# ChocoWu/SeTok

Measured on AMD Instinct MI355X. Metric: images/s SeTok encode (ViT-L/14, 224^2, dyn-k), higher is better.
Workload: dtype bf16; 1 GPU; cfg2: ViT-L/14 224^2 (24 of 24 layers, select_layer=-1 as the reference's launch scripts pass it), dyn-k DPC-kNN (k=64, threshold=0.125), SeTok head 1024/2 heads/ff 4096 -> 4096, mm_in_projector mlp2x_gelu; encode-only; batch_per_gpu=256, global_batch=256, slowest_rank=0

## Files before the change

setok_amd/csrc/attn_seg.hip:

```cpp
#include "lds_mma.h"

namespace {

constexpr int SD = 512;
constexpr int WD = 128;
constexpr int VROW = WD * 2;

__device__ __forceinline__ void attn_seg_big_segment(const bf16* __restrict__ qkv, const int32_t* __restrict__ seg_offsets, bf16* __restrict__ out, int H,
                                                     float scale_log2e, const int s, const int h, float (*Sp)[16 * 64], char (*Vs)[32 * VROW]) {
    const int tid = threadIdx.x, lane = tid & 63;
    const int wave = __builtin_amdgcn_readfirstlane(tid >> 6);
    const int r0 = seg_offsets[s];
    const int n = seg_offsets[s + 1] - r0;
    if (n <= 32) return;
    const int nt = (n + 31) >> 5;
    const int64_t C = (int64_t)H * SD, ld = 3 * C;
    const bf16* qb = qkv + (int64_t)r0 * ld + h * SD + wave * WD;
    const bf16* kb = qb + C;
    const bf16* vb = qb + 2 * C;
    const int qi = lane & 31, hi = lane >> 5;
    const int g16 = lane >> 4, i16 = lane & 15;
    const int tr_row = (i16 >> 2) + 4 * (g16 >> 1);
    const int tr_col = (g16 & 1) * 16 + (i16 & 3) * 4;
    const unsigned vlds = __builtin_amdgcn_readfirstlane((unsigned)(size_t)(__attribute__((address_space(3))) char*)&Vs[0][0]) + wave * (32 * VROW);
    float* mySp = &Sp[wave][0];

    for (int qt = 0; qt < nt; ++qt) {
        const int q = qt * 32 + qi;
        const bf16* qp = qb + (int64_t)min(q, n - 1) * ld + hi * 8;
        bf16x8 qf[8];
#pragma unroll
        for (int ks = 0; ks < 8; ++ks) qf[ks] = *reinterpret_cast<const bf16x8*>(qp + ks * 16);
        f32x16 o[4];
#pragma unroll
        for (int d = 0; d < 4; ++d)
#pragma unroll
            for (int r = 0; r < 16; ++r) o[d][r] = 0.f;
        float m_run = -INFINITY, l_run = 0.f;

        for (int kt = 0; kt < nt; ++kt) {
#pragma unroll
            for (int i = 0; i < 8; ++i) {
                const int p = i * 64 + lane, key = kt * 32 + (p >> 4), c = p & 15;
                const bf16* src = vb + (int64_t)min(key, n - 1) * ld + c * 8;
                lds_dma16(src, vlds + i * 1024);
            }
            f32x16 sp;
#pragma unroll
            for (int r = 0; r < 16; ++r) sp[r] = 0.f;
            const bf16* kp = kb + (int64_t)min(kt * 32 + qi, n - 1) * ld + hi * 8;
            bf16x8 kf[8];
#pragma unroll
            for (int ks = 0; ks < 8; ++ks) kf[ks] = *reinterpret_cast<const bf16x8*>(kp + ks * 16);
#pragma unroll
            for (int ks = 0; ks < 8; ++ks) sp = __builtin_amdgcn_mfma_f32_32x32x16_bf16(kf[ks], qf[ks], sp, 0, 0, 0);
#pragma unroll
            for (int r = 0; r < 16; ++r) mySp[r * 64 + lane] = sp[r];
            __syncthreads();
            float t[16];
#pragma unroll
            for (int r = 0; r < 16; ++r) t[r] = (Sp[0][r * 64 + lane] + Sp[1][r * 64 + lane]) + (Sp[2][r * 64 + lane] + Sp[3][r * 64 + lane]);
            __syncthreads();
            float mx = -INFINITY;
            const bool tail = (kt == nt - 1) && (n & 31);
#pragma unroll
            for (int r = 0; r < 16; ++r) {
                if (tail) { const int key = kt * 32 + (r & 3) + 8 * (r >> 2) + 4 * hi; if (key >= n) t[r] = -INFINITY; }
                mx = fmaxf(mx, t[r]);
            }
            mx = fmaxf(mx, __shfl_xor(mx, 32, 64));
            const float m_new = fmaxf(m_run, mx);
            if (!__all(m_new == m_run)) {
                const float alpha = __builtin_amdgcn_exp2f((m_run - m_new) * scale_log2e);
                l_run *= alpha;
#pragma unroll
                for (int d = 0; d < 4; ++d)
#pragma unroll
                    for (int r = 0; r < 16; ++r) o[d][r] *= alpha;
                m_run = m_new;
            }
            const float mc = m_run * scale_log2e;
            float ls = 0.f;
#pragma unroll
            for (int r = 0; r < 16; ++r) { t[r] = __builtin_amdgcn_exp2f(fmaf(t[r], scale_log2e, -mc)); ls += t[r]; }
            l_run += ls;
            const bf16x8 p0 = pack8(t), p1 = pack8(t + 8);
            asm volatile("s_waitcnt vmcnt(0)" ::: "memory");
            const char* Vw = &Vs[wave][0];
#pragma unroll
            for (int d = 0; d < 4; ++d) {
#pragma unroll
                for (int k2 = 0; k2 < 2; ++k2) {
                    const char* va = Vw + (k2 * 16 + tr_row) * VROW + (d * 32 + tr_col) * 2;
                    o[d] = __builtin_amdgcn_mfma_f32_32x32x16_bf16(lds_read_tr16(va, va + 8 * VROW), k2 == 0 ? p0 : p1, o[d], 0, 0, 0);
                }
            }
            asm volatile("s_waitcnt lgkmcnt(0)" ::: "memory");
        }
        const float l_tot = l_run + __shfl_xor(l_run, 32, 64);
        const float inv = 1.0f / l_tot;
        if (q < n) {
            bf16* op = out + ((int64_t)r0 + q) * C + h * SD + wave * WD;
#pragma unroll
            for (int d = 0; d < 4; ++d)
#pragma unroll
                for (int r4 = 0; r4 < 4; ++r4) {
                    bf16x4 v;
#pragma unroll
                    for (int j = 0; j < 4; ++j) v[j] = (bf16)(o[d][r4 * 4 + j] * inv);
                    *reinterpret_cast<bf16x4*>(op + d * 32 + 8 * r4 + 4 * hi) = v;
                }
        }
    }
}

template <int SPW>
__global__ __launch_bounds__(256) void attn_seg_big_kernel(const bf16* __restrict__ qkv, const int32_t* __restrict__ seg_offsets, int n_segs,
                                                           bf16* __restrict__ out, int H, float scale_log2e) {
    __shared__ __attribute__((aligned(16))) float Sp[4][16 * 64];
    __shared__ __attribute__((aligned(16))) char Vs[4][32 * VROW];
    if constexpr (SPW == 1) {
        attn_seg_big_segment(qkv, seg_offsets, out, H, scale_log2e, blockIdx.x, blockIdx.y, Sp, Vs);
    } else {
        static_assert(SPW == 64, "one lane per segment length");
        const int sl = blockIdx.x * 64 + (threadIdx.x & 63);
        const int nl = sl < n_segs ? seg_offsets[sl + 1] - seg_offsets[sl] : 0;
        unsigned long long m = __ballot(nl > 32);
        while (m) {
            const int b = __builtin_amdgcn_readfirstlane(__ffsll((long long)m) - 1);
            m &= m - 1;
            attn_seg_big_segment(qkv, seg_offsets, out, H, scale_log2e, blockIdx.x * 64 + b, blockIdx.y, Sp, Vs);
            __syncthreads();
        }
    }
}

__global__ __launch_bounds__(256) void attn_seg_small_kernel(const bf16* __restrict__ qkv, const int32_t* __restrict__ seg_offsets, int n_segs,
                                                             bf16* __restrict__ out, int H, float scale_log2e) {
    __shared__ __attribute__((aligned(16))) char Vs[4][32 * VROW];
    const int tid = threadIdx.x, lane = tid & 63;
    const int wave = __builtin_amdgcn_readfirstlane(tid >> 6);
    const int s = blockIdx.x * 4 + wave, h = blockIdx.y;
    if (s >= n_segs) return;
    const int r0 = seg_offsets[s];
    const int n = seg_offsets[s + 1] - r0;
    if (n <= 0 || n > 32) return;
    const int64_t C = (int64_t)H * SD, ld = 3 * C;
    const bf16* qb = qkv + (int64_t)r0 * ld + h * SD;
    const int qi = lane & 31, hi = lane >> 5;
    const int g16 = lane >> 4, i16 = lane & 15;
    const int tr_row = (i16 >> 2) + 4 * (g16 >> 1);
    const int tr_col = (g16 & 1) * 16 + (i16 & 3) * 4;
    const unsigned vlds = __builtin_amdgcn_readfirstlane((unsigned)(size_t)(__attribute__((address_space(3))) char*)&Vs[0][0]) + wave * (32 * VROW);
    const bf16* rowp = qb + (int64_t)min(qi, n - 1) * ld + hi * 8;
    float t[16];
#pragma unroll
    for (int r = 0; r < 16; ++r) t[r] = 0.f;
    f32x16 part[4];
#pragma unroll
    for (int w = 0; w < 4; ++w) {
        bf16x8 qf[8], kf[8];
#pragma unroll
        for (int ks = 0; ks < 8; ++ks) {
            qf[ks] = *reinterpret_cast<const bf16x8*>(rowp + w * WD + ks * 16);
            kf[ks] = *reinterpret_cast<const bf16x8*>(rowp + C + w * WD + ks * 16);
        }
#pragma unroll
        for (int r = 0; r < 16; ++r) part[w][r] = 0.f;
#pragma unroll
        for (int ks = 0; ks < 8; ++ks) part[w] = __builtin_amdgcn_mfma_f32_32x32x16_bf16(kf[ks], qf[ks], part[w], 0, 0, 0);
    }
    float mx = -INFINITY;
#pragma unroll
    for (int r = 0; r < 16; ++r) {
        t[r] = (part[0][r] + part[1][r]) + (part[2][r] + part[3][r]);
        const int key = (r & 3) + 8 * (r >> 2) + 4 * hi;
        if (key >= n) t[r] = -INFINITY;
        mx = fmaxf(mx, t[r]);
    }
    mx = fmaxf(mx, __shfl_xor(mx, 32, 64));
    const float mc = mx * scale_log2e;
    float ls = 0.f;
#pragma unroll
    for (int r = 0; r < 16; ++r) { t[r] = __builtin_amdgcn_exp2f(fmaf(t[r], scale_log2e, -mc)); ls += t[r]; }
    const float inv = 1.0f / (ls + __shfl_xor(ls, 32, 64));
    const bf16x8 p0 = pack8(t), p1 = pack8(t + 8);
    const char* Vw = &Vs[wave][0];
#pragma unroll 1
    for (int w = 0; w < 4; ++w) {
        const bf16* vb = qb + 2 * C + w * WD;
#pragma unroll
        for (int i = 0; i < 8; ++i) {
            const int p = i * 64 + lane, key = p >> 4, c = p & 15;
            const bf16* src = vb + (int64_t)min(key, n - 1) * ld + c * 8;
            lds_dma16(src, vlds + i * 1024);
        }
        asm volatile("s_waitcnt vmcnt(0)" ::: "memory");
        f32x16 o[4];
#pragma unroll
        for (int d = 0; d < 4; ++d) {
#pragma unroll
            for (int r = 0; r < 16; ++r) o[d][r] = 0.f;
#pragma unroll
            for (int k2 = 0; k2 < 2; ++k2) {
                const char* va = Vw + (k2 * 16 + tr_row) * VROW + (d * 32 + tr_col) * 2;
                o[d] = __builtin_amdgcn_mfma_f32_32x32x16_bf16(lds_read_tr16(va, va + 8 * VROW), k2 == 0 ? p0 : p1, o[d], 0, 0, 0);
            }
        }
        asm volatile("s_waitcnt lgkmcnt(0)" ::: "memory");
        if (qi < n) {
            bf16* op = out + ((int64_t)r0 + qi) * C + h * SD + w * WD;
#pragma unroll
            for (int d = 0; d < 4; ++d)
#pragma unroll
                for (int r4 = 0; r4 < 4; ++r4) {
                    bf16x4 v;
#pragma unroll
                    for (int j = 0; j < 4; ++j) v[j] = (bf16)(o[d][r4 * 4 + j] * inv);
                    *reinterpret_cast<bf16x4*>(op + d * 32 + 8 * r4 + 4 * hi) = v;
                }
        }
    }
}

}

int setok_attention_seg_bf16(hipStream_t s, const bf16* qkv, const int32_t* seg_offsets, int n_segs, int max_len, bf16* out, int rows, int H, int Dh, float scale) {
    if (Dh != SD || !seg_offsets || n_segs <= 0 || rows <= 0) return SETOK_EUNSUPPORTED;
    attn_seg_small_kernel<<<dim3(cdiv(n_segs, 4), H), 256, 0, s>>>(qkv, seg_offsets, n_segs, out, H, scale * 1.44269504088896340736f);
    if (max_len > 32) {
        if (n_segs > 2048) attn_seg_big_kernel<64><<<dim3(cdiv(n_segs, 64), H), 256, 0, s>>>(qkv, seg_offsets, n_segs, out, H, scale * 1.44269504088896340736f);
        else attn_seg_big_kernel<1><<<dim3(n_segs, H), 256, 0, s>>>(qkv, seg_offsets, n_segs, out, H, scale * 1.44269504088896340736f);
    }
    SETOK_CHECK_LAUNCH("setok_attention(segments bf16)");
    return SETOK_OK;
}
```

Before: 6345 images/s.

## Restructure small-segment attention with LDS-staged Q/K/V, swizzled layout, persistent grid

Rewrites the small-segment (n<=32) attention kernel to be persistent, with each wave looping over segments picked by ballot from a strided set. Segments of 8 or 16 tokens are handled by a staged path that DMAs Q, K and V rows into XOR-swizzled LDS. Outputs are staged through LDS so global writes are coalesced 16-byte stores, and V loads are overlapped with compute. The goal is to cut wasted loads for short segments, bank conflicts and uncoalesced stores, at the cost of much more complex code, 24KB of LDS per wave, and occupancy pinned at 2 waves per EU.

```diff
diff --git a/setok_amd/csrc/attn_seg.hip b/setok_amd/csrc/attn_seg.hip
--- a/setok_amd/csrc/attn_seg.hip
+++ b/setok_amd/csrc/attn_seg.hip
@@ -135,27 +135,186 @@
     }
 }
 
-__global__ __launch_bounds__(256) void attn_seg_small_kernel(const bf16* __restrict__ qkv, const int32_t* __restrict__ seg_offsets, int n_segs,
-                                                             bf16* __restrict__ out, int H, float scale_log2e) {
-    __shared__ __attribute__((aligned(16))) char Vs[4][32 * VROW];
-    const int tid = threadIdx.x, lane = tid & 63;
-    const int wave = __builtin_amdgcn_readfirstlane(tid >> 6);
-    const int s = blockIdx.x * 4 + wave, h = blockIdx.y;
-    if (s >= n_segs) return;
-    const int r0 = seg_offsets[s];
-    const int n = seg_offsets[s + 1] - r0;
-    if (n <= 0 || n > 32) return;
-    const int64_t C = (int64_t)H * SD, ld = 3 * C;
-    const bf16* qb = qkv + (int64_t)r0 * ld + h * SD;
-    const int qi = lane & 31, hi = lane >> 5;
+constexpr int SMALL_LDS = 24 * 1024;
+
+__device__ __forceinline__ int seg_swz(int row) { return ((row & 3) << 2) | ((row >> 2) & 3); }
+
+template <int NR>
+__device__ __forceinline__ void seg_stage(const char* base, int64_t ldb, int n, unsigned dst, int lane) {
+    constexpr int RPR = NR / 8, LPR = 64 / RPR;
+    const int rl = lane / LPR, pc = lane % LPR;
+#pragma unroll
+    for (int j = 0; j < 8; ++j) {
+        if (j * RPR < n) {
+            const int row = j * RPR + rl;
+            lds_dma16(base + (int64_t)min(row, n - 1) * ldb + ((pc ^ seg_swz(row)) << 4), dst + j * 1024);
+        }
+    }
+}
+
+template <int P, int KS>
+__device__ __forceinline__ void seg_pv(const char* Vb, int sb, int n, int lane, bf16x8 p0, bf16x8 p1, f32x16 (&o)[4]) {
     const int g16 = lane >> 4, i16 = lane & 15;
     const int tr_row = (i16 >> 2) + 4 * (g16 >> 1);
-    const int tr_col = (g16 & 1) * 16 + (i16 & 3) * 4;
-    const unsigned vlds = __builtin_amdgcn_readfirstlane((unsigned)(size_t)(__attribute__((address_space(3))) char*)&Vs[0][0]) + wave * (32 * VROW);
+    const int colb = (g16 & 1) * 32 + (i16 & 3) * 8;
+    const char* ra[KS][2];
+    int sw[KS][2];
+#pragma unroll
+    for (int k2 = 0; k2 < KS; ++k2)
+#pragma unroll
+        for (int u = 0; u < 2; ++u) {
+            const int r = min(k2 * 16 + tr_row + 8 * u, n - 1);
+            ra[k2][u] = Vb + r * P;
+            sw[k2][u] = seg_swz(r);
+        }
+#pragma unroll
+    for (int d = 0; d < 4; ++d) {
+#pragma unroll
+        for (int r = 0; r < 16; ++r) o[d][r] = 0.f;
+        const int b = sb + d * 64 + colb;
+#pragma unroll
+        for (int k2 = 0; k2 < KS; ++k2) {
+            const char* a0 = ra[k2][0] + ((((b >> 4) ^ sw[k2][0]) << 4) | (b & 8));
+            const char* a1 = ra[k2][1] + ((((b >> 4) ^ sw[k2][1]) << 4) | (b & 8));
+            o[d] = __builtin_amdgcn_mfma_f32_32x32x16_bf16(lds_read_tr16(a0, a1), k2 == 0 ? p0 : p1, o[d], 0, 0, 0);
+        }
+    }
+}
+
+template <int PO>
+__device__ __forceinline__ void seg_o_write(const f32x16 (&o)[4], float inv, char* Ob, int sb, int qi, int hi, bool live) {
+    if (live) {
+        char* orow = Ob + qi * PO;
+        const int z = seg_swz(qi);
+#pragma unroll
+        for (int d = 0; d < 4; ++d)
+#pragma unroll
+            for (int r4 = 0; r4 < 4; ++r4) {
+                bf16x4 v;
+#pragma unroll
+                for (int j = 0; j < 4; ++j) v[j] = (bf16)(o[d][r4 * 4 + j] * inv);
+                const int cb = sb + d * 64 + r4 * 16;
+                *reinterpret_cast<bf16x4*>(orow + ((((cb >> 4) ^ z) << 4) | (hi * 8))) = v;
+            }
+    }
+}
+
+template <int PO, int NR>
+__device__ __forceinline__ void seg_o_flush(const char* Ob, bf16* op, int64_t C, int n, int lane) {
+    constexpr int LPR = PO / 16, RPS = 64 / LPR;
+    const int rl = lane / LPR, pc = lane % LPR;
+#pragma unroll
+    for (int j = 0; j < NR / RPS; ++j) {
+        if (j * RPS < n) {
+            const int row = j * RPS + rl;
+            if (row < n) {
+                const bf16x8 v = *reinterpret_cast<const bf16x8*>(Ob + row * PO + ((pc ^ seg_swz(row)) << 4));
+                *reinterpret_cast<bf16x8*>(op + (int64_t)row * C + pc * 8) = v;
+            }
+        }
+    }
+}
+
+template <int LIVE>
+__device__ __forceinline__ float seg_softmax(float* t, int n, int hi, float scale_log2e) {
+    float mx = -INFINITY;
+#pragma unroll
+    for (int r = 0; r < LIVE; ++r) {
+        const int key = (r & 3) + 8 * (r >> 2) + 4 * hi;
+        if (key >= n) t[r] = -INFINITY;
+        mx = fmaxf(mx, t[r]);
+    }
+    mx = fmaxf(mx, __shfl_xor(mx, 32, 64));
+    const float mc = mx * scale_log2e;
+    float ls = 0.f;
+#pragma unroll
+    for (int r = 0; r < LIVE; ++r) { t[r] = __builtin_amdgcn_exp2f(fmaf(t[r], scale_log2e, -mc)); ls += t[r]; }
+#pragma unroll
+    for (int r = LIVE; r < 16; ++r) t[r] = 0.f;
+    return 1.0f / (ls + __shfl_xor(ls, 32, 64));
+}
+
+template <int NR>
+__device__ __forceinline__ void attn_seg_small_staged(const bf16* qb, bf16* ob, int n, int64_t C, float scale_log2e, unsigned lds, char* Lw, int lane) {
+    const char* L = Lw;
+    constexpr int R = NR / 8, SPR = 4 / R, P = SPR * VROW;
+    constexpr unsigned QO = 0, KO = 8192, VO = 16384;
+    const int64_t ldb = 6 * C;
+    const char* qbytes = reinterpret_cast<const char*>(qb);
+    const int qi = lane & 31, hi = lane >> 5;
+    seg_stage<NR>(qbytes, ldb, n, lds + QO, lane);
+    seg_stage<NR>(qbytes + 2 * C, ldb, n, lds + KO, lane);
+    seg_stage<NR>(qbytes + 4 * C, ldb, n, lds + VO, lane);
+    const int row = min(qi, n - 1);
+    const char* fq = L + QO + row * P;
+    const int fz = seg_swz(row);
+    f32x16 part[4];
+#pragma unroll
+    for (int g = 0; g < R; ++g) {
+        asm volatile("s_waitcnt vmcnt(0)" ::: "memory");
+#pragma unroll
+        for (int wl = 0; wl < SPR; ++wl) {
+            const int w = g * SPR + wl;
+            bf16x8 qf[8], kf[8];
+#pragma unroll
+            for (int ks = 0; ks < 8; ++ks) {
+                const int c = ((wl * 16 + ks * 2 + hi) ^ fz) << 4;
+                qf[ks] = *reinterpret_cast<const bf16x8*>(fq + c);
+                kf[ks] = *reinterpret_cast<const bf16x8*>(fq + (KO - QO) + c);
+            }
+#pragma unroll
+            for (int r = 0; r < 16; ++r) part[w][r] = 0.f;
+#pragma unroll
+            for (int ks = 0; ks < 8; ++ks) part[w] = __builtin_amdgcn_mfma_f32_32x32x16_bf16(kf[ks], qf[ks], part[w], 0, 0, 0);
+        }
+        if (R > 1) {
+            asm volatile("s_waitcnt lgkmcnt(0)" ::: "memory");
+            if (g + 1 < R) {
+                seg_stage<NR>(qbytes + (g + 1) * P, ldb, n, lds + QO, lane);
+                seg_stage<NR>(qbytes + 2 * C + (g + 1) * P, ldb, n, lds + KO, lane);
+            } else {
+                seg_stage<NR>(qbytes + 4 * C + P, ldb, n, lds + QO, lane);
+            }
+        }
+    }
+    float t[16];
+#pragma unroll
+    for (int r = 0; r < NR / 2; ++r) t[r] = (part[0][r] + part[1][r]) + (part[2][r] + part[3][r]);
+    const float inv = seg_softmax<NR / 2>(t, n, hi, scale_log2e);
+    const bf16x8 p0 = pack8(t), p1 = pack8(t + 8);
+    const bool live = qi < n;
+    if constexpr (R == 1) {
+#pragma unroll
+        for (int w = 0; w < 4; ++w) {
+            f32x16 o[4];
+            seg_pv<P, 1>(L + VO, w * VROW, n, lane, p0, p1, o);
+            seg_o_write<1024>(o, inv, Lw + QO, w * VROW, qi, hi, live);
+        }
+        seg_o_flush<1024, 8>(L + QO, ob, C, n, lane);
+    } else {
+        f32x16 o0[4], o1[4];
+        seg_pv<P, 1>(L + VO, 0, n, lane, p0, p1, o0);
+        seg_pv<P, 1>(L + VO, VROW, n, lane, p0, p1, o1);
+        asm volatile("s_waitcnt vmcnt(0)" ::: "memory");
+        seg_o_write<512>(o0, inv, Lw + KO, 0, qi, hi, live);
+        seg_o_write<512>(o1, inv, Lw + KO, VROW, qi, hi, live);
+        seg_o_flush<512, 16>(L + KO, ob, C, n, lane);
+        seg_pv<P, 1>(L + QO, 0, n, lane, p0, p1, o0);
+        seg_pv<P, 1>(L + QO, VROW, n, lane, p0, p1, o1);
+        seg_o_write<512>(o0, inv, Lw + KO, 0, qi, hi, live);
+        seg_o_write<512>(o1, inv, Lw + KO, VROW, qi, hi, live);
+        seg_o_flush<512, 16>(L + KO, ob + 2 * WD, C, n, lane);
+    }
+}
+
+__device__ __forceinline__ void attn_seg_small_direct(const bf16* qb, bf16* ob, int n, int64_t C, float scale_log2e, unsigned lds, char* Lw, int lane) {
+    const char* L = Lw;
+    const int64_t ld = 3 * C;
+    const char* vbytes = reinterpret_cast<const char*>(qb + 2 * C);
+    const int qi = lane & 31, hi = lane >> 5;
+#pragma unroll
+    for (int w = 0; w < 3; ++w) seg_stage<32>(vbytes + w * VROW, 2 * ld, n, lds + w * 8192, lane);
     const bf16* rowp = qb + (int64_t)min(qi, n - 1) * ld + hi * 8;
-    float t[16];
-#pragma unroll
-    for (int r = 0; r < 16; ++r) t[r] = 0.f;
     f32x16 part[4];
 #pragma unroll
     for (int w = 0; w < 4; ++w) {
@@ -170,55 +329,60 @@
 #pragma unroll
         for (int ks = 0; ks < 8; ++ks) part[w] = __builtin_amdgcn_mfma_f32_32x32x16_bf16(kf[ks], qf[ks], part[w], 0, 0, 0);
     }
-    float mx = -INFINITY;
-#pragma unroll
-    for (int r = 0; r < 16; ++r) {
-        t[r] = (part[0][r] + part[1][r]) + (part[2][r] + part[3][r]);
-        const int key = (r & 3) + 8 * (r >> 2) + 4 * hi;
-        if (key >= n) t[r] = -INFINITY;
-        mx = fmaxf(mx, t[r]);
-    }
-    mx = fmaxf(mx, __shfl_xor(mx, 32, 64));
-    const float mc = mx * scale_log2e;
-    float ls = 0.f;
-#pragma unroll
-    for (int r = 0; r < 16; ++r) { t[r] = __builtin_amdgcn_exp2f(fmaf(t[r], scale_log2e, -mc)); ls += t[r]; }
-    const float inv = 1.0f / (ls + __shfl_xor(ls, 32, 64));
+    float t[16];
+#pragma unroll
+    for (int r = 0; r < 16; ++r) t[r] = (part[0][r] + part[1][r]) + (part[2][r] + part[3][r]);
+    const float inv = seg_softmax<16>(t, n, hi, scale_log2e);
     const bf16x8 p0 = pack8(t), p1 = pack8(t + 8);
-    const char* Vw = &Vs[wave][0];
-#pragma unroll 1
-    for (int w = 0; w < 4; ++w) {
-        const bf16* vb = qb + 2 * C + w * WD;
-#pragma unroll
-        for (int i = 0; i < 8; ++i) {
-            const int p = i * 64 + lane, key = p >> 4, c = p & 15;
-            const bf16* src = vb + (int64_t)min(key, n - 1) * ld + c * 8;
-            lds_dma16(src, vlds + i * 1024);
-        }
-        asm volatile("s_waitcnt vmcnt(0)" ::: "memory");
-        f32x16 o[4];
-#pragma unroll
-        for (int d = 0; d < 4; ++d) {
-#pragma unroll
-            for (int r = 0; r < 16; ++r) o[d][r] = 0.f;
-#pragma unroll
-            for (int k2 = 0; k2 < 2; ++k2) {
-                const char* va = Vw + (k2 * 16 + tr_row) * VROW + (d * 32 + tr_col) * 2;
-                o[d] = __builtin_amdgcn_mfma_f32_32x32x16_bf16(lds_read_tr16(va, va + 8 * VROW), k2 == 0 ? p0 : p1, o[d], 0, 0, 0);
-            }
-        }
-        asm volatile("s_waitcnt lgkmcnt(0)" ::: "memory");
-        if (qi < n) {
-            bf16* op = out + ((int64_t)r0 + qi) * C + h * SD + w * WD;
-#pragma unroll
-            for (int d = 0; d < 4; ++d)
-#pragma unroll
-                for (int r4 = 0; r4 < 4; ++r4) {
-                    bf16x4 v;
-#pragma unroll
-                    for (int j = 0; j < 4; ++j) v[j] = (bf16)(o[d][r4 * 4 + j] * inv);
-                    *reinterpret_cast<bf16x4*>(op + d * 32 + 8 * r4 + 4 * hi) = v;
-                }
+    const bool live = qi < n;
+    asm volatile("s_waitcnt vmcnt(0)" ::: "memory");
+    f32x16 o0[4], o1[4];
+    seg_pv<VROW, 2>(L, 0, n, lane, p0, p1, o0);
+    asm volatile("s_waitcnt lgkmcnt(0)" ::: "memory");
+    seg_stage<32>(vbytes + 3 * VROW, 2 * ld, n, lds, lane);
+    seg_pv<VROW, 2>(L + 8192, 0, n, lane, p0, p1, o1);
+    seg_o_write<VROW>(o0, inv, Lw + 8192, 0, qi, hi, live);
+    asm volatile("s_waitcnt vmcnt(0)" ::: "memory");
+    seg_o_flush<VROW, 32>(L + 8192, ob, C, n, lane);
+    seg_o_write<VROW>(o1, inv, Lw + 8192, 0, qi, hi, live);
+    seg_o_flush<VROW, 32>(L + 8192, ob + WD, C, n, lane);
+    seg_pv<VROW, 2>(L + 16384, 0, n, lane, p0, p1, o0);
+    seg_o_write<VROW>(o0, inv, Lw + 8192, 0, qi, hi, live);
+    seg_o_flush<VROW, 32>(L + 8192, ob + 2 * WD, C, n, lane);
+    seg_pv<VROW, 2>(L, 0, n, lane, p0, p1, o1);
+    seg_o_write<VROW>(o1, inv, Lw + 8192, 0, qi, hi, live);
+    seg_o_flush<VROW, 32>(L + 8192, ob + 3 * WD, C, n, lane);
+}
+
+constexpr int SMALL_NW = 2;
+constexpr int SMALL_GRID = 768;
+
+__global__ __launch_bounds__(64 * SMALL_NW) __attribute__((amdgpu_waves_per_eu(2, 2))) void attn_seg_small_kernel(const bf16* __restrict__ qkv, const int32_t* __restrict__ seg_offsets, int n_segs,
+                                                             bf16* __restrict__ out, int H, float scale_log2e) {
+    __shared__ __attribute__((aligned(16))) char Ls[SMALL_NW][SMALL_LDS];
+    const int tid = threadIdx.x, lane = tid & 63;
+    const int wave = __builtin_amdgcn_readfirstlane(tid >> 6);
+    const int h = blockIdx.y, G = gridDim.x;
+    const int64_t C = (int64_t)H * SD;
+    const unsigned lds = __builtin_amdgcn_readfirstlane((unsigned)(size_t)(__attribute__((address_space(3))) char*)&Ls[0][0]) + wave * SMALL_LDS;
+    char* L = &Ls[wave][0];
+    for (int q0 = blockIdx.x; q0 * SMALL_NW < n_segs; q0 += 64 * G) {
+        const int64_t sl = ((int64_t)q0 + (int64_t)lane * G) * SMALL_NW + wave;
+        int r0l = 0, nl = 0;
+        if (sl < n_segs) { r0l = seg_offsets[sl]; nl = seg_offsets[sl + 1] - r0l; }
+        unsigned long long m = __ballot(nl >= 1 && nl <= 32);
+        while (m) {
+            const int b = __builtin_amdgcn_readfirstlane(__ffsll((long long)m) - 1);
+            m &= m - 1;
+            const int r0 = __builtin_amdgcn_readlane(r0l, b), n = __builtin_amdgcn_readlane(nl, b);
+            const bf16* qb = qkv + (int64_t)r0 * 3 * C + h * SD;
+            bf16* ob = out + (int64_t)r0 * C + h * SD;
+            asm volatile("s_waitcnt lgkmcnt(0)" ::: "memory");
+            int ln = lane;
+            asm volatile("" : "+v"(ln));
+            if (n <= 8) attn_seg_small_staged<8>(qb, ob, n, C, scale_log2e, lds, L, ln);
+            else if (n <= 16) attn_seg_small_staged<16>(qb, ob, n, C, scale_log2e, lds, L, ln);
+            else attn_seg_small_direct(qb, ob, n, C, scale_log2e, lds, L, ln);
         }
     }
 }
@@ -227,7 +391,7 @@
 
 int setok_attention_seg_bf16(hipStream_t s, const bf16* qkv, const int32_t* seg_offsets, int n_segs, int max_len, bf16* out, int rows, int H, int Dh, float scale) {
     if (Dh != SD || !seg_offsets || n_segs <= 0 || rows <= 0) return SETOK_EUNSUPPORTED;
-    attn_seg_small_kernel<<<dim3(cdiv(n_segs, 4), H), 256, 0, s>>>(qkv, seg_offsets, n_segs, out, H, scale * 1.44269504088896340736f);
+    attn_seg_small_kernel<<<dim3(min(cdiv(n_segs, SMALL_NW), SMALL_GRID), H), 64 * SMALL_NW, 0, s>>>(qkv, seg_offsets, n_segs, out, H, scale * 1.44269504088896340736f);
     if (max_len > 32) {
         if (n_segs > 2048) attn_seg_big_kernel<64><<<dim3(cdiv(n_segs, 64), H), 256, 0, s>>>(qkv, seg_offsets, n_segs, out, H, scale * 1.44269504088896340736f);
         else attn_seg_big_kernel<1><<<dim3(n_segs, H), 256, 0, s>>>(qkv, seg_offsets, n_segs, out, H, scale * 1.44269504088896340736f);
```

Result: no change. 6360 images/s (median of 6 runs) (+0.2%).
